# qcraftai/pillarnext

Measured on AMD Instinct MI355X. Metric: frames/s PillarNeXt-B nuScenes 300k-pt cloud (inference, end-to-end), higher is better.
Workload: dtype bf16

## Files before the change

include/pnx.h:

```cpp
#ifndef PNX_H
#define PNX_H

#include <stddef.h>
#include <stdint.h>

#ifdef __cplusplus
extern "C" {
#endif

typedef void* pnx_stream_t;

typedef enum pnx_status {
  PNX_OK = 0,
  PNX_ERR_INVALID = -1,
  PNX_ERR_UNSUPPORTED = -2,
  PNX_ERR_WORKSPACE = -3,
  PNX_ERR_HIP = -4
} pnx_status;

typedef enum pnx_dtype { PNX_F32 = 0, PNX_BF16 = 1, PNX_F16 = 2 } pnx_dtype;
typedef enum pnx_layout {
  PNX_NHWC = 0,
  PNX_NCHW = 1
} pnx_layout;
// ... 83 lines not shown

int pnx_bias_act_mask(const void* x, const void* residual, const float* bias, const uint8_t* mask, void* out, int64_t sites,
                      int32_t channels, int32_t dtype, int32_t relu, pnx_stream_t stream);
int pnx_sum_bias_act(const void* const* srcs, int32_t n_src, const float* bias, void* out, int64_t sites, int32_t channels, int32_t dtype,
                     int32_t relu, pnx_stream_t stream);
int pnx_deconv2x2_bf16(const void* x, const void* wfrag, const float* bias, void* y, int32_t batch, int32_t h, int32_t w, int32_t cin, int32_t cout,
                       int32_t relu, pnx_stream_t stream);
int pnx_deconv2x2_f16(const void* x, const void* wfrag, const float* bias, void* y, int32_t batch, int32_t h, int32_t w, int32_t cin, int32_t cout,
                       int32_t relu, pnx_stream_t stream);
int pnx_conv3x3_bf16(const void* x, const void* wfrag, const float* bias, const void* residual, const uint8_t* mask, void* y, int32_t batch,
                     int32_t h, int32_t w, int32_t cin, int32_t cout, int32_t stride, int32_t relu, uint8_t* row_dirty, const int32_t* tile_list,
                     const int32_t* tile_count, pnx_stream_t stream);
int pnx_conv3x3_f16(const void* x, const void* wfrag, const float* bias, const void* residual, const uint8_t* mask, void* y, int32_t batch,
                    int32_t h, int32_t w, int32_t cin, int32_t cout, int32_t stride, int32_t relu, uint8_t* row_dirty, const int32_t* tile_list,
                    const int32_t* tile_count, pnx_stream_t stream);
size_t pnx_conv3x3_wgrad_workspace_bytes(int32_t cin, int32_t cout);
int pnx_conv3x3_wgrad_bf16(const void* x, const void* dy, const uint8_t* mask, float* dw, int32_t batch, int32_t h, int32_t w, int32_t cin, int32_t cout,
                           int32_t stride, void* workspace, size_t workspace_bytes, pnx_stream_t stream);
int pnx_conv3x3_wgrad_x3(const void* x_hi, const void* x_lo, const void* dy_hi, const void* dy_lo, const uint8_t* mask, float* dw, int32_t batch, int32_t h,
                         int32_t w, int32_t cin, int32_t cout, int32_t stride, void* workspace, size_t workspace_bytes, pnx_stream_t stream);
int pnx_conv3x3_wgrad_x6(const void* x_hi, const void* x_mid, const void* x_lo, const void* dy_hi, const void* dy_mid, const void* dy_lo, const uint8_t* mask,
                         float* dw, int32_t batch, int32_t h, int32_t w, int32_t cin, int32_t cout, int32_t stride, void* workspace, size_t workspace_bytes,
                         pnx_stream_t stream);
int pnx_conv3x3_pack_weights(const void* w, int32_t dtype, int32_t cout, int32_t cin, int32_t transposed, void* wfrag, pnx_stream_t stream);
int pnx_conv3x3_tile_rows(int32_t cin, int32_t cout, int32_t stride);
int pnx_conv_tile_list(const uint8_t* mask, const uint8_t* const* row_dirty, int32_t n_dirty, int32_t batch, int32_t h, int32_t w, int32_t tile_rows,
                       int32_t* tile_list, int32_t* tile_count, pnx_stream_t stream);
int pnx_sephead_out_bf16(const void* x, const void* wfrag, const float* bias, void* y, int32_t batch, int32_t h, int32_t w, int32_t n_branch,
                         pnx_stream_t stream);
int pnx_sephead_out_f16(const void* x, const void* wfrag, const float* bias, void* y, int32_t batch, int32_t h, int32_t w, int32_t n_branch,
// ... 204 lines not shown
```

pillarnext_amd/_lib.py:

```python
import ctypes
import os

_HERE = os.path.dirname(os.path.abspath(__file__))
LIB_PATH = os.environ.get("PNX_LIB") or os.path.join(_HERE, "libpnx_hip.so")

PNX_F32, PNX_BF16, PNX_F16 = 0, 1, 2
PNX_NHWC, PNX_NCHW = 0, 1


class PnxError(RuntimeError):
    pass


class PnxGeom(ctypes.Structure):
    _fields_ = [("pc_min", ctypes.c_float * 3), ("voxel", ctypes.c_float * 3), ("gx", ctypes.c_int32), ("gy", ctypes.c_int32)]


PNX_GROUP_VOXEL, PNX_GROUP_PILLAR_CLAMP, PNX_GROUP_CYLINDER_CLAMP = 0, 1, 2


class PnxGroupGeom(ctypes.Structure):
    _fields_ = [("min", ctypes.c_float * 3), ("voxel", ctypes.c_float * 3), ("grid", ctypes.c_int32 * 3), ("mode", ctypes.c_int32),
                ("prefilter", ctypes.c_int32), ("keep_min", ctypes.c_float * 3), ("keep_max", ctypes.c_float * 3)]

# ... 56 lines not shown
    "pnx_deconv2x2_f16": (ctypes.c_int, [_vp, _vp, _vp, _vp, _i32, _i32, _i32, _i32, _i32, _i32, _vp]),
    "pnx_sephead_out_bf16": (ctypes.c_int, [_vp, _vp, _vp, _vp, _i32, _i32, _i32, _i32, _vp]),
    "pnx_sephead_out_f16": (ctypes.c_int, [_vp, _vp, _vp, _vp, _i32, _i32, _i32, _i32, _vp]),
    "pnx_masked_bn_blocks": (_i32, []),
    "pnx_masked_bn_reduce": (ctypes.c_int, [_vp, _i32, _i32, _vp, _vp]),
    "pnx_masked_bn_finalize": (ctypes.c_int, [_vp, _i32, _vp, _vp, _vp, ctypes.c_double, ctypes.c_double, _vp, _vp, _vp, _vp, _vp, _vp, _vp, _vp, _vp]),
    "pnx_masked_bn_bwd_finalize": (ctypes.c_int, [_vp, _vp, _i32, _vp, _vp, _vp, _vp, _vp, _vp]),
    "pnx_masked_bn_stats": (ctypes.c_int, [_vp, _i32, _vp, _i64, _i32, _vp, _vp, _vp]),
    "pnx_masked_bn_apply": (ctypes.c_int, [_vp, _vp, _i32, _vp, _i64, _i32, _vp, _vp, _i32, _vp, _vp]),
    "pnx_masked_bn_bwd_stats": (ctypes.c_int, [_vp, _vp, _vp, _i32, _vp, _i64, _i32, _vp, _vp, _vp, _vp, _i32, _vp, _vp]),
    "pnx_masked_bn_bwd_apply": (ctypes.c_int, [_vp, _vp, _vp, _i32, _vp, _i64, _i32, _vp, _vp, _vp, _vp, _i32, _vp, _vp, _vp, _vp, _vp]),
    "pnx_sephead_lazy_bf16": (ctypes.c_int, [_vp, _i32, _vp, _i32, _i32, _vp, _vp, _i32, _vp, _vp]),
    "pnx_sephead_lazy_f16": (ctypes.c_int, [_vp, _i32, _vp, _i32, _i32, _vp, _vp, _i32, _vp, _vp]),
    "pnx_conv3x3_bf16": (ctypes.c_int, [_vp, _vp, _vp, _vp, _vp, _vp, _i32, _i32, _i32, _i32, _i32, _i32, _i32, _vp, _vp, _vp, _vp]),
    "pnx_conv3x3_f16": (ctypes.c_int, [_vp, _vp, _vp, _vp, _vp, _vp, _i32, _i32, _i32, _i32, _i32, _i32, _i32, _vp, _vp, _vp, _vp]),
    "pnx_conv3x3_tile_rows": (ctypes.c_int, [_i32, _i32, _i32]),
    "pnx_conv3x3_pack_weights": (ctypes.c_int, [_vp, _i32, _i32, _i32, _i32, _vp, _vp]),
    "pnx_conv3x3_wgrad_workspace_bytes": (_sz, [_i32, _i32]),
    "pnx_conv3x3_wgrad_bf16": (ctypes.c_int, [_vp, _vp, _vp, _vp, _i32, _i32, _i32, _i32, _i32, _i32, _vp, _sz, _vp]),
    "pnx_conv3x3_wgrad_x3": (ctypes.c_int, [_vp, _vp, _vp, _vp, _vp, _vp, _i32, _i32, _i32, _i32, _i32, _i32, _vp, _sz, _vp]),
    "pnx_conv3x3_wgrad_x6": (ctypes.c_int, [_vp, _vp, _vp, _vp, _vp, _vp, _vp, _vp, _i32, _i32, _i32, _i32, _i32, _i32, _vp, _sz, _vp]),
    "pnx_conv3x3_dgrad_s2_bf16": (ctypes.c_int, [_vp, _vp, _vp, _vp, _i32, _i32, _i32, _i32, _i32, _vp]),
    "pnx_conv3x3_dgrad_s2_x3": (ctypes.c_int, [_vp, _vp, _vp, _vp, _vp, _vp, _i32, _i32, _i32, _i32, _i32, _vp]),
    "pnx_conv3x3_dgrad_s2_x6": (ctypes.c_int, [_vp, _vp, _vp, _vp, _vp, _vp, _vp, _vp, _i32, _i32, _i32, _i32, _i32, _vp]),
    "pnx_conv3x3_smallk": (ctypes.c_int, [_vp, _vp, _vp, _vp, _i32, _i32, _i32, _i32, _i32, _i32, _vp]),
    "pnx_conv3x3_smallk_wgrad_workspace_bytes": (_sz, [_i32]),
    "pnx_conv3x3_smallk_wgrad": (ctypes.c_int, [_vp, _vp, _vp, _vp, _i32, _i32, _i32, _i32, _i32, _i32, _vp, _sz, _vp]),
    "pnx_conv_tile_list": (ctypes.c_int, [_vp, _vp, _i32, _i32, _i32, _i32, _i32, _vp, _vp, _vp]),
    "pnx_mask_pool3": (ctypes.c_int, [_vp, _i32, _i32, _i32, _i32, _vp, _vp]),
    "pnx_split_f32": (ctypes.c_int, [_vp, _vp, _vp, _i64, _vp, _i32, _vp]),
    "pnx_conv3x3_x3": (ctypes.c_int, [_vp, _vp, _vp, _vp, _vp, _vp, _vp, _i32, _i32, _i32, _i32, _i32, _i32, _vp]),
# ... 96 lines not shown
```

pillarnext_amd/csrc/conv3x3.hip:

```cpp
#include "pnx_common.h"

namespace {

#include "conv_tile.h"

template <int CIN, int COUT, int STRIDE, bool W_LDS>
__global__ __launch_bounds__(256, 2) void k_conv3x3(const uint16_t* __restrict__ x, const uint4* __restrict__ wfrag,
                                                 const float* __restrict__ bias, const uint16_t* __restrict__ res,
                                                 const uint8_t* __restrict__ mask, uint16_t* __restrict__ y, int B, int H, int W, int Ho,
                                                 int Wo, int relu, uint8_t* __restrict__ row_dirty) {
  constexpr int CB = CIN / 16, MT = COUT / 32, KSTEPS = 9 * CB;
  constexpr int NT = (MT <= 2) ? 4 : 2;
  extern __shared__ uint4 s_w[];
  const int lane = threadIdx.x & 63, wv = threadIdx.x >> 6;
  const int px = lane & 31, kb = lane >> 5;
  if (W_LDS) {
    for (int i = threadIdx.x; i < KSTEPS * MT * 64; i += 256) s_w[i] = wfrag[i];
    __syncthreads();
  }
  const int tiles_x = (Wo + 31) >> 5, tiles_y = (Ho + NT - 1) / NT;
  const int64_t n_tiles = (int64_t)B * tiles_y * tiles_x;
  for (int64_t tile = (int64_t)blockIdx.x * 4 + wv; tile < n_tiles; tile += (int64_t)gridDim.x * 4) {
    const int tx = (int)(tile % tiles_x);
    const int ty = (int)((tile / tiles_x) % tiles_y);
// ... 267 lines not shown
  k_tile_list<<<(unsigned)((n_tiles + 15) / 16), 256, 0, st>>>(mask, ds, batch, h, w, tile_rows, tile_list, tile_count);
  PNX_LAUNCH_CHECK();
  return PNX_OK;
}
int pnx_conv_tile_list(const uint8_t* mask, const uint8_t* const* row_dirty, int32_t n_dirty, int32_t batch, int32_t h, int32_t w, int32_t tile_rows,
                       int32_t* tile_list, int32_t* tile_count, pnx_stream_t stream) {
  return conv_tile_list_impl(mask, row_dirty, n_dirty, batch, h, w, tile_rows, tile_list, tile_count, stream, true);
}
int pnx_conv_tile_list_prezeroed(const uint8_t* mask, const uint8_t* const* row_dirty, int32_t n_dirty, int32_t batch, int32_t h, int32_t w, int32_t tile_rows,
                                 int32_t* tile_list, int32_t* tile_count, pnx_stream_t stream) {
  return conv_tile_list_impl(mask, row_dirty, n_dirty, batch, h, w, tile_rows, tile_list, tile_count, stream, false);
}

#endif

int PNX_CONV_FN(pnx_conv3x3)(const void* x, const void* wfrag, const float* bias, const void* residual, const uint8_t* mask, void* y, int32_t batch,
                     int32_t h, int32_t w, int32_t cin, int32_t cout, int32_t stride, int32_t relu, uint8_t* row_dirty, const int32_t* tile_list,
                     const int32_t* tile_count, pnx_stream_t stream) {
  PNX_REQUIRE((tile_list == nullptr) == (tile_count == nullptr), PNX_ERR_INVALID, "tile_list and tile_count come together");
  PNX_REQUIRE(tile_list == nullptr || (mask != nullptr && pnx_conv3x3_tile_rows(cin, cout, stride) > 0), PNX_ERR_INVALID,
              "a tile list needs a mask and a kernel that takes one (pnx_conv3x3_tile_rows)");
  PNX_REQUIRE(x && wfrag && bias && y && batch > 0 && h > 0 && w > 0, PNX_ERR_INVALID, "bad arguments");
  PNX_REQUIRE(stride == 1 || stride == 2, PNX_ERR_UNSUPPORTED, "stride %d", stride);
  PNX_REQUIRE(row_dirty == nullptr || mask != nullptr, PNX_ERR_INVALID, "row_dirty needs an active-site mask");
  PNX_REQUIRE((((uintptr_t)x | (uintptr_t)y | (uintptr_t)wfrag | (uintptr_t)bias | (uintptr_t)residual) & 15) == 0, PNX_ERR_INVALID,
              "16-byte alignment required");
  const int ho = (h + 2 - 3) / stride + 1, wo = (w + 2 - 3) / stride + 1;
  hipStream_t st = (hipStream_t)stream;
  const ConvArgs a = {(const uint16_t*)x, (const uint4*)wfrag, bias, (const uint16_t*)residual, mask, (uint16_t*)y, batch, h, w, relu, row_dirty, tile_list,
                      tile_count, st};
  if (stride == 1 && getenv("PNX_CONV_DIRECT") == nullptr) {
    static const int pc_mode = getenv("PNX_CONV_PC") != nullptr ? atoi(getenv("PNX_CONV_PC")) : 1;
    static const int pack_mode = getenv("PNX_CONV_PACK") != nullptr ? atoi(getenv("PNX_CONV_PACK")) : 3;
    if (pc_mode != 0) {
      if (cin == 64 && cout == 64) return launch_pc<64, 64>(a, (pack_mode & 2) != 0);
      if (residual == nullptr && (pc_mode & 4)) {
        if (cin == 64 && cout == 320) return launch_pc<64, 320>(a);
        if (cin == 64 && cout == 384) return launch_pc<64, 384>(a);
        if (cin == 64 && cout == 448) return launch_pc<64, 448>(a);
      }
      if (pc_mode & 2) {
        if (cin == 128 && cout == 128) return launch_pc<128, 128>(a);
        if (cin == 256 && cout == 256) return launch_pc<256, 256>(a);
      }
    }
    if (cin == 64 && cout == 64) return launch_lds<64>(a);
    const bool pack = (pack_mode & 1) != 0;
    if (cin == 128 && cout == 128) return launch_ldsx<128, 128>(a, pack);
    if (cin == 256 && cout == 64) return launch_ldsx<256, 64>(a);
    if (cin == 256 && cout == 256) return launch_ldsx<256, 256>(a, pack);
// ... 5 lines not shown
    if (cin == 64 && cout == 128) return launch_s2<64, 128, 1>(x, wfrag, bias, mask, y, batch, h, w, ho, wo, relu, row_dirty, st);
    if (cin == 128 && cout == 256) return launch_s2<128, 256, 1>(x, wfrag, bias, mask, y, batch, h, w, ho, wo, relu, row_dirty, st);
    if (cin == 256 && cout == 256) return launch_s2<256, 256, 1>(x, wfrag, bias, mask, y, batch, h, w, ho, wo, relu, row_dirty, st);
  }
#define PNX_CONV_CASE(CI, CO)                             \
  if (cin == CI && cout == CO) {                          \
    if (stride == 1) return launch<CI, CO, 1>(a, ho, wo); \
    return launch<CI, CO, 2>(a, ho, wo);                  \
  }
  PNX_CONV_CASE(64, 64)
  PNX_CONV_CASE(64, 128)
  PNX_CONV_CASE(128, 128)
#undef PNX_CONV_CASE
  pnx_set_error("pnx_conv3x3: no kernel for %d -> %d channels", cin, cout);
  return PNX_ERR_UNSUPPORTED;
}

#ifndef PNX_CONV_F16
}
namespace {
#include "conv_dgrad_s2.h"

template <int NP>
int dgrad_s2_impl(const char* name, PnxPieces<NP> g, PnxPieces<NP> wfrag_t, const uint8_t* mask_in, void* dx, int32_t batch, int32_t h, int32_t w, int32_t cin,
                  int32_t cout, pnx_stream_t stream) {
  PNX_REQUIRE(g.complete() && wfrag_t.complete() && mask_in && dx && batch > 0 && h > 0 && w > 0, PNX_ERR_INVALID, "%s: bad arguments", name);
  PNX_REQUIRE(((g.bits() | wfrag_t.bits() | (uintptr_t)dx) & 15) == 0, PNX_ERR_INVALID, "16-byte alignment required");
  hipStream_t st = (hipStream_t)stream;
  if (cin == 64 && cout == 128) return launch_dgrad_s2<128, 64, NP>(g, wfrag_t, mask_in, dx, batch, h, w, st);
  if (cin == 128 && cout == 256) return launch_dgrad_s2<256, 128, NP>(g, wfrag_t, mask_in, dx, batch, h, w, st);
// ... 94 lines not shown
```

pillarnext_amd/csrc/conv_pc.h:

```cpp
#pragma once

__device__ __forceinline__ void pc_barrier_lds() { asm volatile("s_waitcnt lgkmcnt(0)\n\ts_barrier" ::: "memory"); }
__device__ __forceinline__ void pc_barrier_all() { asm volatile("s_waitcnt vmcnt(0) lgkmcnt(0)\n\ts_barrier" ::: "memory"); }

#ifdef PNX_CONV_TIMERS
#define PC_T_DECL unsigned long long pc_T[8] = {0, 0, 0, 0, 0, 0, 0, 0}; unsigned long long pc_tk = __builtin_amdgcn_s_memtime();
#define PC_TOCK(k)                                               \
  {                                                              \
    const unsigned long long _n = __builtin_amdgcn_s_memtime();  \
    pc_T[k] += _n - pc_tk;                                       \
    pc_tk = _n;                                                  \
  }
#define PC_T_FLUSH                                                   \
  if ((threadIdx.x & 63) == 0) {                                     \
    for (int k = 0; k < 8; k++) atomicAdd(&g_conv_T[k], pc_T[k]);    \
  }
#else
#define PC_T_DECL
#define PC_TOCK(k)
#define PC_T_FLUSH
#endif

template <int NR, int CIN, int COUT, bool HAS_RES, int NRG, int NSLOT, int SLOT_N, int NP = 1>
__device__ __forceinline__ void pc_rows(const uint4* __restrict__ s_ring, int& g, const uint4* __restrict__ wfrag, const uint4* __restrict__ wfrag2,
// ... 148 lines not shown
      transpose_row32(pk, lane);
      int l = lane;
      asm volatile("" : "+v"(l));
      const int cj = code(j);
#pragma unroll
      for (int d = 0; d < 2; d++) {
        const int P = 16 * d + (l >> 2);
        const int pc = __builtin_amdgcn_ds_bpermute(P << 2, cj);
        if (P < n_g[j]) *reinterpret_cast<uint4*>(yp + pc_pix_off64(pc, W) + (uint32_t)((l & 3) * 16)) = pk[d];
      }
    }
  }
  PC_TOCK(3)
}

template <int CIN, int COUT, bool HAS_RES, int NP = 1, bool PACK = false>
__global__ __launch_bounds__(768, 3) void k_conv3x3_pc(const uint16_t* __restrict__ x, const uint16_t* __restrict__ x2, const uint4* __restrict__ wfrag,
                                                       const uint4* __restrict__ wfrag2, const float* __restrict__ bias,
                                                       const uint16_t* __restrict__ res, const uint8_t* __restrict__ mask, uint16_t* __restrict__ y,
                                                       int B, int H, int W, int relu, uint8_t* __restrict__ row_dirty, int slot,
                                                       const int32_t* __restrict__ tlist, const int32_t* __restrict__ tcount,
                                                       const uint16_t* __restrict__ x3 = nullptr, const uint4* __restrict__ wfrag3 = nullptr) {
  constexpr bool X3 = NP == 2, F32 = NP > 1;
  constexpr int TH = CIN == 64 ? 16 : 8;
  constexpr int NRG = TH / 4, NCG = 8 / NRG, PASS_C = NCG * 32, NPASS = COUT / PASS_C, NSLAB = CIN / 64;
  constexpr int NSLOT = CIN == 64 ? 2 : 3, DEPTH = NSLOT - 1;
  constexpr int NFILL = F32 ? NPASS * NSLAB * NP : CIN == 64 ? 1 : NPASS * NSLAB;
  constexpr int YS = F32 ? 2 : 1;
  static_assert(!F32 || (!HAS_RES && (CIN > 64 || NPASS == 1)), "fp32 product: no residual; one pass when the tile is filled once per source");
  constexpr int SLOT_N = (TH + 2) * LDS_HW * 8;
  static_assert(COUT % PASS_C == 0 && CIN % 64 == 0, "passes of NCG x 32 output channels over 64-channel input slabs");
  static_assert(!PACK || (CIN == 64 && COUT == 64 && NP == 1), "the packed-pixel form serves the bf16 / f16 64 -> 64 layers");
  __shared__ uint4 s_ring[NSLOT * SLOT_N];
  __shared__ uint16_t s_list[PACK ? 4 * TH * 32 : 1];
  __shared__ int4 s_tile[4];
  __shared__ uint32_t s_rowmask[4][TH];
  __shared__ int4 s_drow[4][NRG];
  __shared__ uint4 s_dmask[4][NRG];
// ... 10 lines not shown
#pragma unroll
    for (int i = 0; i < 5; i++) {
      const int col = 8 * i + (lane >> 3), k = lane & 7;
      colv[i] = col;
      voff[i] = (uint32_t)(col * CIN + ((k ^ lds_swz(col)) * 8)) * 2u;
    }
    typedef __attribute__((address_space(1))) const void* gptr_t;
    typedef __attribute__((address_space(3))) void* lptr_t;

    auto tile_index = [&](int n) -> int64_t {
      const int64_t idx = (n < 3 || slot < 0) ? (int64_t)blockIdx.x + (int64_t)n * gridDim.x : (int64_t)s_tick[n & 3] + 3 * (int64_t)gridDim.x;
      return tile_at(tlist, idx, n_tiles);
    };
    uint32_t mb[TH / 2];
    uint32_t dirty = 0;
    auto load_meta = [&](int64_t t) {
#pragma unroll
      for (int k = 0; k < TH / 2; k++) mb[k] = 0;
      dirty = 0;
      if (t < 0) return;
      const int tx = (int)(t % tiles_x), ty = (int)((t / tiles_x) % tiles_y), b = (int)(t / ((int64_t)tiles_x * tiles_y));
      const int ox = tx * 32 + (lane & 31);
#pragma unroll
      for (int k = 0; k < TH / 2; k++) {
        const int oy = ty * TH + 2 * k + (lane >> 5);
        if (ox < W && oy < H) mb[k] = mask != nullptr ? (uint32_t)mask[((int64_t)b * H + oy) * W + ox] : 1u;
      }
      const int oy2 = ty * TH + lane;
      if (lane < TH && oy2 < H) dirty = row_dirty != nullptr ? (uint32_t)row_dirty[((int64_t)b * H + oy2) * tiles_x + tx] : 1u;
    };

    int n = 0, f = 0, nf = 0, g = 0;
    int64_t t_next = tile_index(0);
    load_meta(t_next);
    int cb = 0, cy0 = 0, cx0 = 0;
    uint32_t am = 0;

    auto advance = [&]() -> bool {
      const int64_t t = t_next;
      if (t < 0) {
        if (pw == 0 && lane == 0) s_tile[n & 3] = make_int4(-1, 0, 0, 0);
        return false;
      }
      const int tx = (int)(t % tiles_x), ty = (int)((t / tiles_x) % tiles_y);
// ... 4 lines not shown
      int n_px = 0;
#pragma unroll
      for (int k = 0; k < TH / 2; k++) {
        const unsigned long long bal = __ballot(mb[k] != 0);
        const uint32_t lo = (uint32_t)bal, hi = (uint32_t)(bal >> 32);
        if constexpr (PACK) {
          if (pw == 0 && mb[k] != 0)
            s_list[(n & 3) * (TH * 32) + n_px + __popcll(bal & ((1ull << lane) - 1ull))] = (uint16_t)(((2 * k + (lane >> 5)) << 5) | (lane & 31));
          n_px += __popcll(bal);
        }
        if (lane == 2 * k) my_rm = lo;
        if (lane == 2 * k + 1) my_rm = hi;
        am |= (lo != 0 ? 1u : 0u) << (2 * k) | (hi != 0 ? 1u : 0u) << (2 * k + 1);
      }
      const uint32_t was = (uint32_t)__ballot(dirty != 0) & ((1u << TH) - 1u);
      if (pw == 0) {
        if (lane < TH) s_rowmask[n & 3][lane] = my_rm;
        if (lane == 0) s_tile[n & 3] = make_int4(cb, cy0, cx0, (int)(am | (uint32_t)n_px << 16));
        if (lane < NRG * 4) {
          uint32_t rest = am;
          for (int k = 0; k < lane && rest; k++) rest &= rest - 1;
          const int row = rest != 0 ? __builtin_ctz(rest) : -1;
          const uint32_t m = row >= 0 ? s_rowmask[n & 3][row] : 0u;
          reinterpret_cast<int*>(&s_drow[n & 3][lane % NRG])[lane / NRG] = row;
          reinterpret_cast<uint32_t*>(&s_dmask[n & 3][lane % NRG])[lane / NRG] = m;
        }
      }
      if (slot >= 0 && pw == 0 && lane == 0) s_tick[(n + 3) & 3] = atomicAdd(&g_tile_ctr[slot][0], 1u);
      t_next = tile_index(n + 1);
      load_meta(t_next);
// ... 28 lines not shown
      n++;
      return true;
    };

    auto next_fill = [&]() -> bool {
      if (f == nf && !advance()) return false;
      if (am != 0) {
        const int sl = f % NSLAB;
        uint4* dstslot = s_ring + (g % NSLOT) * SLOT_N;
        const uint16_t* xs = X3 && (f / NSLAB) % 2 == 1 ? x2 : x;
        if constexpr (NP == 3) {
          const int q = (f / NSLAB) % 3;
          xs = q == 0 ? x3 : q == 1 ? x2 : x;
        }
        const uint16_t* xt = xs + (((int64_t)cb * H + (cy0 - 1)) * W + (cx0 - 1)) * CIN + 64 * sl;
        bool col_ok[5];
#pragma unroll
        for (int i = 0; i < 5; i++) col_ok[i] = (unsigned)(cx0 - 1 + colv[i]) < (unsigned)W && (i < 4 || lane < 16);
#pragma unroll 1
        for (int r = pw; r < TH + 2; r += 4) {
          const int iy = cy0 - 1 + r;
          const bool row_ok = iy >= 0 && iy < H;
          const char* rowp = reinterpret_cast<const char*>(xt + (int64_t)r * W * CIN);
#pragma unroll
          for (int i = 0; i < 5; i++) {
            if (row_ok && col_ok[i]) {
              __builtin_amdgcn_global_load_lds((gptr_t)(rowp + voff[i]), (lptr_t)(dstslot + r * LDS_HW * 8 + 64 * i), 16, 0, 0);
            } else if (i < 4 || lane < 16) {
              dstslot[r * LDS_HW * 8 + 64 * i + lane] = make_uint4(0, 0, 0, 0);
            }
          }
        }
      }
      f++;
      g++;
// ... 95 lines not shown
      default: PC_ROWS(4); break;
    }
#undef PC_ROWS
  }
  if (threadIdx.x == 0) sched_done(slot);
  PC_T_FLUSH
}

template <int CIN, int COUT>
int launch_pc(const ConvArgs& a, bool pack = false) {
  constexpr int TH = CIN == 64 ? 16 : 8;
  int64_t nb = (int64_t)a.B * ((a.H + TH - 1) / TH) * ((a.W + 31) / 32);
  if (nb > 256) nb = 256;
  const int slot = a.mask != nullptr ? next_sched_slot() : -1;
  if constexpr (CIN == 64 && COUT == 64) {
    if (pack && a.mask != nullptr) {
      if (a.res != nullptr)
        k_conv3x3_pc<64, 64, true, 1, true><<<(unsigned)nb, 768, 0, a.st>>>(a.x, nullptr, a.wfrag, nullptr, a.bias, a.res, a.mask, a.y, a.B, a.H, a.W, a.relu,
                                                                          a.row_dirty, slot, a.tlist, a.tcount);
      else
        k_conv3x3_pc<64, 64, false, 1, true><<<(unsigned)nb, 768, 0, a.st>>>(a.x, nullptr, a.wfrag, nullptr, a.bias, nullptr, a.mask, a.y, a.B, a.H, a.W, a.relu,
                                                                           a.row_dirty, slot, a.tlist, a.tcount);
      PNX_LAUNCH_CHECK();
      return PNX_OK;
    }
  }
  if (a.res != nullptr)
    k_conv3x3_pc<CIN, COUT, true><<<(unsigned)nb, 768, 0, a.st>>>(a.x, nullptr, a.wfrag, nullptr, a.bias, a.res, a.mask, a.y, a.B, a.H, a.W, a.relu, a.row_dirty,
                                                                slot, a.tlist, a.tcount);
  else
// ... 19 lines not shown
```

pillarnext_amd/csrc/conv_tile.h:

```cpp
#pragma once

typedef float v16f __attribute__((ext_vector_type(16)));
typedef float f32x2 __attribute__((ext_vector_type(2)));

#ifdef PNX_CONV_F16
typedef _Float16 el8 __attribute__((ext_vector_type(8)));
typedef _Float16 el2 __attribute__((ext_vector_type(2)));
#define PNX_MFMA32(a, b, c) __builtin_amdgcn_mfma_f32_32x32x16_f16(a, b, c, 0, 0, 0)
#define PNX_MFMA16(a, b, c) __builtin_amdgcn_mfma_f32_16x16x32_f16(a, b, c, 0, 0, 0)
#define PNX_CONV_FN(name) name##_f16
__device__ __forceinline__ uint32_t el_lo_bits(uint32_t w) { return __float_as_uint((float)__builtin_bit_cast(el2, w)[0]); }
__device__ __forceinline__ uint32_t el_hi_bits(uint32_t w) { return __float_as_uint((float)__builtin_bit_cast(el2, w)[1]); }
#else
typedef __bf16 el8 __attribute__((ext_vector_type(8)));
typedef __bf16 el2 __attribute__((ext_vector_type(2)));
#define PNX_MFMA32(a, b, c) __builtin_amdgcn_mfma_f32_32x32x16_bf16(a, b, c, 0, 0, 0)
#define PNX_MFMA16(a, b, c) __builtin_amdgcn_mfma_f32_16x16x32_bf16(a, b, c, 0, 0, 0)
#define PNX_CONV_FN(name) name##_bf16
__device__ __forceinline__ uint32_t el_lo_bits(uint32_t w) { return w << 16; }
__device__ __forceinline__ uint32_t el_hi_bits(uint32_t w) { return w & 0xffff0000u; }
#endif
__device__ __forceinline__ uint32_t pack_el(float lo, float hi) {
  const f32x2 v = {lo, hi};
  return __builtin_bit_cast(uint32_t, __builtin_convertvector(v, el2));
// ... 147 lines not shown
      }
    }
}

struct ConvArgs {
  const uint16_t* x;
  const uint4* wfrag;
  const float* bias;
  const uint16_t* res;
  const uint8_t* mask;
  uint16_t* y;
  int B, H, W, relu;
  uint8_t* row_dirty;
  const int32_t *tlist, *tcount;
  hipStream_t st;
};
```

pillarnext_amd/csrc/enqueue.hip:

```cpp
#include "pnx_common.h"

extern "C" int pnx_conv_tile_list_prezeroed(const uint8_t* mask, const uint8_t* const* row_dirty, int32_t n_dirty, int32_t batch, int32_t h, int32_t w,
                                            int32_t tile_rows, int32_t* tile_list, int32_t* tile_count, pnx_stream_t stream);

namespace {

__global__ __launch_bounds__(256) void k_lazy_cells(const int64_t* __restrict__ order, const int32_t* __restrict__ seg_len, const int64_t* __restrict__ list_key_off,
                                                    int32_t pre_max, int64_t n, int64_t* __restrict__ local) {
  const int64_t i = (int64_t)blockIdx.x * blockDim.x + threadIdx.x;
  if (i >= n) return;
  const int64_t s = i / pre_max;
  const int32_t j = (int32_t)(i - s * pre_max);
  local[i] = j < seg_len[s] ? order[i] - list_key_off[s] : 0;
}

struct ZeroRanges {
  uint32_t* p[8];
  int64_t end[8];
  int n;
};
__global__ __launch_bounds__(256) void k_zero_ranges(ZeroRanges z) {
  const int64_t total = z.end[z.n - 1];
  for (int64_t i = (int64_t)blockIdx.x * 256 + threadIdx.x; i < total; i += (int64_t)gridDim.x * 256) {
    int r = 0;
// ... 14 lines not shown
  z.p[z.n] = (uint32_t*)p;
  z.end[z.n] = (z.n ? z.end[z.n - 1] : 0) + words;
  z.n++;
}

int run_op(const pnx_op& o, hipStream_t st) {
  const int32_t* i = o.i;
  const void* const* p = o.p;
  switch (o.kind) {
    case PNX_OP_MASK_POOL3:
      return pnx_mask_pool3((const uint8_t*)p[0], i[0], i[1], i[2], i[3], (uint8_t*)p[1], st);
    case PNX_OP_TILE_LIST:
      PNX_REQUIRE(i[0] >= 0 && i[0] <= 8, PNX_ERR_INVALID, "tile list over %d row_dirty arrays (at most 8)", i[0]);
      return pnx_conv_tile_list_prezeroed((const uint8_t*)p[0], (const uint8_t* const*)&p[3], i[0], i[1], i[2], i[3], i[4], (int32_t*)p[1], (int32_t*)p[2], st);
    case PNX_OP_CONV3X3:
      return (i[7] == PNX_F16 ? pnx_conv3x3_f16 : pnx_conv3x3_bf16)(p[0], p[1], (const float*)p[2], p[3], (const uint8_t*)p[4], (void*)p[5], i[0], i[1], i[2],
                                                                    i[3], i[4], i[5], i[6], (uint8_t*)p[6], (const int32_t*)p[7], (const int32_t*)p[8], st);
    case PNX_OP_DECONV2X2:
      return (i[6] == PNX_F16 ? pnx_deconv2x2_f16 : pnx_deconv2x2_bf16)(p[0], p[1], (const float*)p[2], (void*)p[3], i[0], i[1], i[2], i[3], i[4], i[5], st);
    case PNX_OP_SEPHEAD_OUT:
      return (i[4] == PNX_F16 ? pnx_sephead_out_f16 : pnx_sephead_out_bf16)(p[0], p[1], (const float*)p[2], (void*)p[3], i[0], i[1], i[2], i[3], st);
    default:
      pnx_set_error("unknown op kind %d", o.kind);
      return PNX_ERR_INVALID;
  }
}

}

extern "C" int pnx_enqueue(const pnx_op* ops, int32_t n_ops, pnx_stream_t stream) {
  PNX_REQUIRE(ops != nullptr && n_ops >= 0, PNX_ERR_INVALID, "pnx_enqueue: bad arguments");
  hipStream_t st = (hipStream_t)stream;
// ... 81 lines not shown
```

pillarnext_amd/models.py:

```python
import copy
import inspect
import os
import weakref

import numpy as np

import torch
import torch.nn.functional as F
from torch import nn

from . import ops
from .plan import Dyn, LaunchPlan


def _spconv_weight_to_conv2d(w, conv):
    want = tuple(conv.weight.shape)
    co, ci, kh, kw = want
    layout = getattr(conv, "assume_layout", None)
    if layout == "dense":
        if tuple(w.shape) != want:
            raise RuntimeError(f"dense-layout checkpoint holds {tuple(w.shape)} for Conv2d {want}")
        return w
    if layout == "spconv":
        if tuple(w.shape) != (co, kh, kw, ci):
# ... 951 lines not shown
            y = F.conv2d(x, self.weight, None, self.stride, self.padding, self.dilation)
        if not y.is_contiguous(memory_format=torch.channels_last):
            y = y.contiguous(memory_format=torch.channels_last)
        if post_residual is not None:
            return ops.bias_act_mask_(y, self.bias, mask, post_residual, 2 if self.relu else 0)
        return ops.bias_act_mask_(y, self.bias, mask, residual, self.relu)


class _HipConv3x3(nn.Module):

    def __init__(self, weight, bias, stride=1, dtype=torch.bfloat16):
        super().__init__()
        self.cout, self.cin, self.stride = weight.shape[0], weight.shape[1], int(stride)
        self.register_buffer("wfrag", ops.conv3x3_pack_weights(weight, dtype=dtype))
        self.register_buffer("bias", bias.float().contiguous())
    def forward(self, x, mask=None, residual=None, out=None, tiles=None, plan=None):
        call = ops.conv3x3_masked if plan is None else plan.conv3x3
        return call(x, self.wfrag, self.bias, self.cout, self.stride, mask, residual, True, out=out, tiles=tiles if self.stride == 1 else None)


class _HipDeconv2x2(nn.Module):

    def __init__(self, weight, bias, relu=True, dtype=torch.bfloat16):
        super().__init__()
        self.cout, self.relu = weight.shape[1], relu
        self.register_buffer("wfrag", ops.deconv2x2_pack_weights(weight, dtype=dtype))
        self.register_buffer("bias", bias.float().contiguous())

    def forward(self, x, mask=None, residual=None, out=None, plan=None):
        if plan is None:
            return ops.deconv2x2(x, self.wfrag, self.bias, self.cout, self.relu)
        return plan.deconv2x2(x, self.wfrag, self.bias, self.cout, out, self.relu)

# ... 68 lines not shown
        return getattr(self.pend, name)


class FusedPillarNeXt(nn.Module):

    def __init__(self, det, dtype=torch.bfloat16, hip_conv=None):
        super().__init__()
        import os

        if hip_conv is None:
            hip_conv = os.environ.get("PNX_HIP_CONV", "1") != "0"
        self._ws = {}
        self.use_plan = os.environ.get("PNX_PLAN", "1") != "0"
        self.sparse_ws = os.environ.get("PNX_SPARSE_WS", "1") != "0"
        self.tile_lists = os.environ.get("PNX_TILE_LISTS", "1") != "0"
        self.decode_on_side_stream = os.environ.get("PNX_DECODE_STREAM", "1") != "0"
        self.reader = det.reader
        self.post_processing = det.post_processing
        self.head_ref = det.head
        self.dtype = dtype
        self._decoder = None
        bb = det.backbone
        self.stages = nn.ModuleList()
        self.stage_meta = []
        for blk in bb.blocks:
            mods = nn.ModuleList()
            first = blk[0]
            w, b = _fold_bn(first.conv.weight, first.norm)
            mods.append(_backbone_conv(w, b, first.stride, first.kernel_size // 2, dtype, hip_conv))
            for rb in list(blk)[1:]:
# ... 143 lines not shown
            if lazy:
                packed_out.append(LazyTask(t, up))
            elif packed_out is not None:
                packed_out.append(t)
            else:
                d, o = {}, 0
                for nme, k in zip(names, outs_n):
                    d[nme] = t[:, o:o + k]
                    o += k
                preds.append(d)
        mark("head")
        return preds

    def _backbone(self, x, mask, plan=None, mark=lambda name: None, taps=None):
        for si, (mods, (stride, subm)) in enumerate(zip(self.stages, self.stage_meta)):
            if not subm:
                mask = ops.mask_pool3(mask, stride) if plan is None else plan.mask_pool3(mask, ops.mask_pool3_out(mask, stride), stride)
            ws, k = self._stage_workspace(si, mods, mask), 0
            tiles = self._stage_tiles(si, mods, mask, ws, plan)

            def run(m, inp, res=None):
                nonlocal k
                if ws is None or not isinstance(m, _HipConv3x3):
                    assert plan is None
                    return m(inp, mask, residual=res)
                k += 1
                return m(inp, mask, residual=res, out=ws[(k - 1) % 3], tiles=tiles, plan=plan)

            x = run(mods[0], x)
            for j in range(1, len(mods), 2):
                y = run(mods[j], x)
                x = run(mods[j + 1], y, x)
            mark(f"backbone.stage{si}")
            if taps is not None:
                taps[f"stage{si}"] = x
        return x, mask

    def _head(self, x, lazy, plan=None):
        c1s, c2s = (self.lazy_conv1, self.lazy_conv2) if lazy else (self.task_conv1, self.task_conv2)

        def run(m, inp, out):
            return m(inp) if plan is None else m(inp, out=out, plan=plan)

        o_sh, outs = None, [(None, None, None)] * len(c1s)
        if plan is not None:
            def new(c, s):
                return torch.empty((x.shape[0], c, s * x.shape[2], s * x.shape[3]), dtype=self.dtype, device=x.device, memory_format=torch.channels_last)
# ... 173 lines not shown
```

pillarnext_amd/ops.py:

```python
import ctypes

import torch

from . import _lib
from ._lib import PNX_BF16, PNX_F16, PNX_F32, PNX_NCHW, PNX_NHWC, PnxError, check, lib, ptr, stream_ptr

_DT = {torch.float32: PNX_F32, torch.bfloat16: PNX_BF16, torch.float16: PNX_F16}


def _need_cuda(t, name):
    if not t.is_cuda:
        raise PnxError(f"{name} must be a CUDA (ROCm) tensor; the PillarNeXt hot path has no CPU implementation")
    if not t.is_contiguous():
        raise PnxError(f"{name} must be contiguous")


class Workspace:

    def __init__(self):
        self.buf = None

    def get(self, nbytes, device):
        if self.buf is None or self.buf.numel() < nbytes or self.buf.device != device:
            self.buf = torch.empty(int(nbytes * 1.25) + 256, dtype=torch.uint8, device=device)
# ... 614 lines not shown

def _conv3x3_dims(x, wfrag, cout, stride, mask, residual, out, cuda=False):
    xs = _half_nhwc(x, "conv3x3", cuda=cuda)
    if wfrag.dtype != xs.dtype or (residual is not None and _like(residual).dtype != xs.dtype):
        raise PnxError("conv3x3: weights / residual of another dtype than the input")
    B, ci, H, W = xs.shape
    Ho, Wo = _out_hw(H, W, stride)
    if out is not None:
        y, dirty = out
        if (tuple(_half_nhwc(y, "conv3x3 output", xs.dtype).shape) != (B, cout, Ho, Wo)
                or (dirty is not None and (mask is None or tuple(dirty.shape) != (B, Ho, (Wo + 31) // 32)))):
            raise PnxError("conv3x3: output / workspace of the wrong shape (a workspace needs a mask)")
    return B, H, W, ci, _DT[xs.dtype], Ho, Wo


def conv3x3_masked(x, wfrag, bias, cout, stride=1, mask=None, residual=None, relu=True, out=None, tiles=None):
    B, H, W, ci, _, Ho, Wo = _conv3x3_dims(x, wfrag, cout, stride, mask, residual, out, cuda=True)
    y, dirty = out if out is not None else (torch.empty((B, cout, Ho, Wo), dtype=x.dtype, device=x.device, memory_format=torch.channels_last), None)
    tl, tc = tiles if tiles is not None else (None, None)
    check(_conv_fn("conv3x3", x.dtype)(ptr(x), ptr(wfrag), ptr(bias), ptr(residual), ptr(mask), ptr(y), B, H, W, ci, cout, stride, 1 if relu else 0,
                                       ptr(dirty), ptr(tl), ptr(tc), stream_ptr()), "pnx_conv3x3")
    return y


def _i3(v):
    return (ctypes.c_int32 * 3)(*[int(a) for a in v])


class Sp3Index:

    def __init__(self, batch, grid, device):
        self.batch, self.grid = int(batch), tuple(int(g) for g in grid)
        self.nbytes = lib().pnx_sp3_index_bytes(self.batch, _i3(self.grid))
        if self.nbytes == 0:
            raise PnxError(f"sparse3d: bad grid {self.batch} x {self.grid}")
        self.buf = torch.empty((self.nbytes,), dtype=torch.uint8, device=device)
# ... 354 lines not shown
```

pillarnext_amd/plan.py:

```python
import ctypes

from . import ops
from ._lib import PnxError, check, lib, stream_ptr

OP_MASK_POOL3, OP_TILE_LIST, OP_CONV3X3, OP_DECONV2X2, OP_SEPHEAD_OUT = 1, 2, 3, 4, 5


class PnxOp(ctypes.Structure):
    _fields_ = [("kind", ctypes.c_int32), ("i", ctypes.c_int32 * 9), ("p", ctypes.c_void_p * 11)]


assert ctypes.sizeof(PnxOp) == 128, "pnx_op layout drifted (include/pnx.h)"


class Dyn:

    def __init__(self, name, like):
        self.name, self.like = name, like


class LaunchPlan:
    def __init__(self):
        self._ops, self._keep, self._dyn, self._arr = [], [], {}, None

# ... 16 lines not shown
                op.p[k] = a.data_ptr()
                self._keep.append(a)
        self._ops.append(op)

    def mask_pool3(self, mask_in, mask_out, stride):
        self._add(OP_MASK_POOL3, [*ops._like(mask_in).shape, stride], [mask_in, ops.mask_pool3_out(mask_in, stride, mask_out)])
        return mask_out

    def tile_list(self, mask, dirties, tile_rows, out):
        if len(dirties) > 8:
            raise PnxError("tile_list: an entry has room for 8 row_dirty arrays")
        tl, tc = ops.conv_tile_buffers(mask, tile_rows, out)
        self._add(OP_TILE_LIST, [len(dirties), *ops._like(mask).shape, tile_rows], [mask, tl, tc] + list(dirties))
        return out

    def conv3x3(self, x, wfrag, bias, cout, stride=1, mask=None, residual=None, relu=True, out=None, tiles=None):
        B, H, W, ci, dt, _, _ = ops._conv3x3_dims(x, wfrag, cout, stride, mask, residual, out)
        tl, tc = tiles if tiles is not None else (None, None)
        self._add(OP_CONV3X3, [B, H, W, ci, cout, stride, 1 if relu else 0, dt], [x, wfrag, bias, residual, mask, *out, tl, tc])
        return out[0]

    def deconv2x2(self, x, wfrag, bias, cout, y, relu=True):
        B, H, W, ci, dt = ops._conv_dims("deconv2x2", x, wfrag, y, cout, 2)
        self._add(OP_DECONV2X2, [B, H, W, ci, cout, 1 if relu else 0, dt], [x, wfrag, bias, y])
        return y

    def sephead_out(self, x, wfrag, bias, y):
        B, H, W, ci, dt = ops._conv_dims("sephead_out", x, wfrag, y, 16, 1)
        self._add(OP_SEPHEAD_OUT, [B, H, W, ci // 64, dt], [x, wfrag, bias, y])
        return y

    def freeze(self):
        self._arr = (PnxOp * max(len(self._ops), 1))(*self._ops)
        self._bound = {}
# ... 23 lines not shown
```

Measured before the change: 758.8.

## Skip gathering inactive input pixels in stage-0 64->64 sparse conv via input mask

Adds an input active-site mask path to the 64->64 pillar conv kernel. Halo pixels whose input is inactive are zero-filled in LDS instead of loaded from global memory, and whole input rows that no active output row needs are skipped. This is meant to cut redundant global-to-LDS traffic for sparse stage-0 feature maps, at the cost of an extra mask read and ballots per tile. The row-skip part also applies to the existing non-input-mask path, but the input-mask path is wired only for stage 0 and is disabled by default through PNX_STAGE0_IN_MASK=0.

Result: no change. 761.6 (median of 6 runs) (+0.4%).

```diff
diff --git a/include/pnx.h b/include/pnx.h
--- a/include/pnx.h
+++ b/include/pnx.h
@@ -121,6 +121,12 @@
 int pnx_conv3x3_f16(const void* x, const void* wfrag, const float* bias, const void* residual, const uint8_t* mask, void* y, int32_t batch,
                     int32_t h, int32_t w, int32_t cin, int32_t cout, int32_t stride, int32_t relu, uint8_t* row_dirty, const int32_t* tile_list,
                     const int32_t* tile_count, pnx_stream_t stream);
+int pnx_conv3x3_in_bf16(const void* x, const void* wfrag, const float* bias, const void* residual, const uint8_t* mask, const uint8_t* in_mask, void* y,
+                        int32_t batch, int32_t h, int32_t w, int32_t cin, int32_t cout, int32_t stride, int32_t relu, uint8_t* row_dirty,
+                        const int32_t* tile_list, const int32_t* tile_count, pnx_stream_t stream);
+int pnx_conv3x3_in_f16(const void* x, const void* wfrag, const float* bias, const void* residual, const uint8_t* mask, const uint8_t* in_mask, void* y,
+                       int32_t batch, int32_t h, int32_t w, int32_t cin, int32_t cout, int32_t stride, int32_t relu, uint8_t* row_dirty,
+                       const int32_t* tile_list, const int32_t* tile_count, pnx_stream_t stream);
 size_t pnx_conv3x3_wgrad_workspace_bytes(int32_t cin, int32_t cout);
 int pnx_conv3x3_wgrad_bf16(const void* x, const void* dy, const uint8_t* mask, float* dw, int32_t batch, int32_t h, int32_t w, int32_t cin, int32_t cout,
                            int32_t stride, void* workspace, size_t workspace_bytes, pnx_stream_t stream);
diff --git a/pillarnext_amd/_lib.py b/pillarnext_amd/_lib.py
--- a/pillarnext_amd/_lib.py
+++ b/pillarnext_amd/_lib.py
@@ -94,7 +94,9 @@
     "pnx_sephead_lazy_f16": (ctypes.c_int, [_vp, _i32, _vp, _i32, _i32, _vp, _vp, _i32, _vp, _vp]),
     "pnx_conv3x3_bf16": (ctypes.c_int, [_vp, _vp, _vp, _vp, _vp, _vp, _i32, _i32, _i32, _i32, _i32, _i32, _i32, _vp, _vp, _vp, _vp]),
     "pnx_conv3x3_f16": (ctypes.c_int, [_vp, _vp, _vp, _vp, _vp, _vp, _i32, _i32, _i32, _i32, _i32, _i32, _i32, _vp, _vp, _vp, _vp]),
-    "pnx_conv3x3_tile_rows": (ctypes.c_int, [_i32, _i32, _i32]),
+    "pnx_conv3x3_in_bf16": (ctypes.c_int, [_vp, _vp, _vp, _vp, _vp, _vp, _vp, _i32, _i32, _i32, _i32, _i32, _i32, _i32, _vp, _vp, _vp, _vp]),
+    "pnx_conv3x3_in_f16": (ctypes.c_int, [_vp, _vp, _vp, _vp, _vp, _vp, _vp, _i32, _i32, _i32, _i32, _i32, _i32, _i32, _vp, _vp, _vp, _vp]),
+    "pnx_conv3x3_tile_rows":(ctypes.c_int, [_i32, _i32, _i32]),
     "pnx_conv3x3_pack_weights": (ctypes.c_int, [_vp, _i32, _i32, _i32, _i32, _vp, _vp]),
     "pnx_conv3x3_wgrad_workspace_bytes": (_sz, [_i32, _i32]),
     "pnx_conv3x3_wgrad_bf16": (ctypes.c_int, [_vp, _vp, _vp, _vp, _i32, _i32, _i32, _i32, _i32, _i32, _vp, _sz, _vp]),
diff --git a/pillarnext_amd/csrc/conv3x3.hip b/pillarnext_amd/csrc/conv3x3.hip
--- a/pillarnext_amd/csrc/conv3x3.hip
+++ b/pillarnext_amd/csrc/conv3x3.hip
@@ -305,10 +305,11 @@
 
 #endif
 
-int PNX_CONV_FN(pnx_conv3x3)(const void* x, const void* wfrag, const float* bias, const void* residual, const uint8_t* mask, void* y, int32_t batch,
-                     int32_t h, int32_t w, int32_t cin, int32_t cout, int32_t stride, int32_t relu, uint8_t* row_dirty, const int32_t* tile_list,
-                     const int32_t* tile_count, pnx_stream_t stream) {
+int PNX_CONV_FN(pnx_conv3x3_in)(const void* x, const void* wfrag, const float* bias, const void* residual, const uint8_t* mask, const uint8_t* in_mask,
+                        void* y, int32_t batch, int32_t h, int32_t w, int32_t cin, int32_t cout, int32_t stride, int32_t relu, uint8_t* row_dirty,
+                        const int32_t* tile_list, const int32_t* tile_count, pnx_stream_t stream) {
   PNX_REQUIRE((tile_list == nullptr) == (tile_count == nullptr), PNX_ERR_INVALID, "tile_list and tile_count come together");
+  PNX_REQUIRE(in_mask == nullptr || mask != nullptr, PNX_ERR_INVALID, "in_mask needs an active-site mask");
   PNX_REQUIRE(tile_list == nullptr || (mask != nullptr && pnx_conv3x3_tile_rows(cin, cout, stride) > 0), PNX_ERR_INVALID,
               "a tile list needs a mask and a kernel that takes one (pnx_conv3x3_tile_rows)");
   PNX_REQUIRE(x && wfrag && bias && y && batch > 0 && h > 0 && w > 0, PNX_ERR_INVALID, "bad arguments");
@@ -319,12 +320,17 @@
   const int ho = (h + 2 - 3) / stride + 1, wo = (w + 2 - 3) / stride + 1;
   hipStream_t st = (hipStream_t)stream;
   const ConvArgs a = {(const uint16_t*)x, (const uint4*)wfrag, bias, (const uint16_t*)residual, mask, (uint16_t*)y, batch, h, w, relu, row_dirty, tile_list,
-                      tile_count, st};
+                      tile_count, st, nullptr};
   if (stride == 1 && getenv("PNX_CONV_DIRECT") == nullptr) {
     static const int pc_mode = getenv("PNX_CONV_PC") != nullptr ? atoi(getenv("PNX_CONV_PC")) : 1;
     static const int pack_mode = getenv("PNX_CONV_PACK") != nullptr ? atoi(getenv("PNX_CONV_PACK")) : 3;
     if (pc_mode != 0) {
-      if (cin == 64 && cout == 64) return launch_pc<64, 64>(a, (pack_mode & 2) != 0);
+      if (cin == 64 && cout == 64) {
+        static const bool use_in_mask = getenv("PNX_CONV_IN_MASK") == nullptr || atoi(getenv("PNX_CONV_IN_MASK")) != 0;
+        ConvArgs ai = a;
+        ai.in_mask = use_in_mask ? in_mask : nullptr;
+        return launch_pc<64, 64>(ai, (pack_mode & 2) != 0);
+      }
       if (residual == nullptr && (pc_mode & 4)) {
         if (cin == 64 && cout == 320) return launch_pc<64, 320>(a);
         if (cin == 64 && cout == 384) return launch_pc<64, 384>(a);
@@ -360,6 +366,12 @@
 #undef PNX_CONV_CASE
   pnx_set_error("pnx_conv3x3: no kernel for %d -> %d channels", cin, cout);
   return PNX_ERR_UNSUPPORTED;
+}
+
+int PNX_CONV_FN(pnx_conv3x3)(const void* x, const void* wfrag, const float* bias, const void* residual, const uint8_t* mask, void* y, int32_t batch,
+                     int32_t h, int32_t w, int32_t cin, int32_t cout, int32_t stride, int32_t relu, uint8_t* row_dirty, const int32_t* tile_list,
+                     const int32_t* tile_count, pnx_stream_t stream) {
+  return PNX_CONV_FN(pnx_conv3x3_in)(x, wfrag, bias, residual, mask, nullptr, y, batch, h, w, cin, cout, stride, relu, row_dirty, tile_list, tile_count, stream);
 }
 
 #ifndef PNX_CONV_F16
diff --git a/pillarnext_amd/csrc/conv_pc.h b/pillarnext_amd/csrc/conv_pc.h
--- a/pillarnext_amd/csrc/conv_pc.h
+++ b/pillarnext_amd/csrc/conv_pc.h
@@ -186,14 +186,16 @@
   PC_TOCK(3)
 }
 
-template <int CIN, int COUT, bool HAS_RES, int NP = 1, bool PACK = false>
+template <int CIN, int COUT, bool HAS_RES, int NP = 1, bool PACK = false, bool INM = false>
 __global__ __launch_bounds__(768, 3) void k_conv3x3_pc(const uint16_t* __restrict__ x, const uint16_t* __restrict__ x2, const uint4* __restrict__ wfrag,
                                                        const uint4* __restrict__ wfrag2, const float* __restrict__ bias,
                                                        const uint16_t* __restrict__ res, const uint8_t* __restrict__ mask, uint16_t* __restrict__ y,
                                                        int B, int H, int W, int relu, uint8_t* __restrict__ row_dirty, int slot,
                                                        const int32_t* __restrict__ tlist, const int32_t* __restrict__ tcount,
-                                                       const uint16_t* __restrict__ x3 = nullptr, const uint4* __restrict__ wfrag3 = nullptr) {
+                                                       const uint16_t* __restrict__ x3 = nullptr, const uint4* __restrict__ wfrag3 = nullptr,
+                                                       const uint8_t* __restrict__ in_mask = nullptr) {
   constexpr bool X3 = NP == 2, F32 = NP > 1;
+  static_assert(!INM || (CIN == 64 && COUT == 64 && NP == 1), "the input's active set is used by the bf16 / f16 64 -> 64 layers");
   constexpr int TH = CIN == 64 ? 16 : 8;
   constexpr int NRG = TH / 4, NCG = 8 / NRG, PASS_C = NCG * 32, NPASS = COUT / PASS_C, NSLAB = CIN / 64;
   constexpr int NSLOT = CIN == 64 ? 2 : 3, DEPTH = NSLOT - 1;
@@ -234,10 +236,17 @@
     };
     uint32_t mb[TH / 2];
     uint32_t dirty = 0;
+    constexpr int NIR = INM ? (TH + 2 + 3) / 4 : 1;
+    [[maybe_unused]] uint32_t ib[NIR];
+    [[maybe_unused]] unsigned long long iw[NIR];
     auto load_meta = [&](int64_t t) {
 #pragma unroll
       for (int k = 0; k < TH / 2; k++) mb[k] = 0;
       dirty = 0;
+      if constexpr (INM) {
+#pragma unroll
+        for (int j = 0; j < NIR; j++) ib[j] = 0;
+      }
       if (t < 0) return;
       const int tx = (int)(t % tiles_x), ty = (int)((t / tiles_x) % tiles_y), b = (int)(t / ((int64_t)tiles_x * tiles_y));
       const int ox = tx * 32 + (lane & 31);
@@ -248,6 +257,14 @@
       }
       const int oy2 = ty * TH + lane;
       if (lane < TH && oy2 < H) dirty = row_dirty != nullptr ? (uint32_t)row_dirty[((int64_t)b * H + oy2) * tiles_x + tx] : 1u;
+      if constexpr (INM) {
+        const int ix = tx * 32 - 1 + lane;
+#pragma unroll
+        for (int j = 0; j < NIR; j++) {
+          const int r = pw + 4 * j, iy = ty * TH - 1 + r;
+          if (r < TH + 2 && lane < 34 && (unsigned)ix < (unsigned)W && (unsigned)iy < (unsigned)H) ib[j] = (uint32_t)in_mask[((int64_t)b * H + iy) * W + ix];
+        }
+      }
     };
 
     int n = 0, f = 0, nf = 0, g = 0;
@@ -282,6 +299,20 @@
         am |= (lo != 0 ? 1u : 0u) << (2 * k) | (hi != 0 ? 1u : 0u) << (2 * k + 1);
       }
       const uint32_t was = (uint32_t)__ballot(dirty != 0) & ((1u << TH) - 1u);
+      if constexpr (INM) {
+#pragma unroll
+        for (int j = 0; j < NIR; j++) iw[j] = __ballot(ib[j] != 0);
+        const uint32_t need = am | am << 1 | am << 2;
+        uint4* dstslot = s_ring + (g % NSLOT) * SLOT_N;
+#pragma unroll
+        for (int j = 0; j < NIR; j++) {
+          const int r = pw + 4 * j;
+          if (r >= TH + 2 || ((need >> r) & 1u) == 0) continue;
+#pragma unroll
+          for (int i = 0; i < 5; i++)
+            if (((iw[j] >> colv[i]) & 1ull) == 0 && (i < 4 || lane < 16)) dstslot[r * LDS_HW * 8 + 64 * i + lane] = make_uint4(0, 0, 0, 0);
+        }
+      }
       if (pw == 0) {
         if (lane < TH) s_rowmask[n & 3][lane] = my_rm;
         if (lane == 0) s_tile[n & 3] = make_int4(cb, cy0, cx0, (int)(am | (uint32_t)n_px << 16));
@@ -340,11 +371,28 @@
           xs = q == 0 ? x3 : q == 1 ? x2 : x;
         }
         const uint16_t* xt = xs + (((int64_t)cb * H + (cy0 - 1)) * W + (cx0 - 1)) * CIN + 64 * sl;
+        const uint32_t need = CIN == 64 && NP == 1 ? am | am << 1 | am << 2 : 0xffffffffu;
+        if constexpr (INM) {
+#pragma unroll
+          for (int j = 0; j < NIR; j++) {
+            const int r = pw + 4 * j;
+            if (r >= TH + 2 || ((need >> r) & 1u) == 0 || iw[j] == 0) continue;
+            const char* rowp = reinterpret_cast<const char*>(xt + (int64_t)r * W * CIN);
+#pragma unroll
+            for (int i = 0; i < 5; i++)
+              if ((iw[j] >> colv[i]) & 1ull)
+                __builtin_amdgcn_global_load_lds((gptr_t)(rowp + voff[i]), (lptr_t)(dstslot + r * LDS_HW * 8 + 64 * i), 16, 0, 0);
+          }
+          f++;
+          g++;
+          return true;
+        }
         bool col_ok[5];
 #pragma unroll
         for (int i = 0; i < 5; i++) col_ok[i] = (unsigned)(cx0 - 1 + colv[i]) < (unsigned)W && (i < 4 || lane < 16);
 #pragma unroll 1
         for (int r = pw; r < TH + 2; r += 4) {
+          if (((need >> r) & 1u) == 0) continue;
           const int iy = cy0 - 1 + r;
           const bool row_ok = iy >= 0 && iy < H;
           const char* rowp = reinterpret_cast<const char*>(xt + (int64_t)r * W * CIN);
@@ -470,6 +518,19 @@
   if (nb > 256) nb = 256;
   const int slot = a.mask != nullptr ? next_sched_slot() : -1;
   if constexpr (CIN == 64 && COUT == 64) {
+    if (a.in_mask != nullptr && a.mask != nullptr) {
+#define PC_INM(RES_, PACK_)                                                                                                                                  \
+  k_conv3x3_pc<64, 64, RES_, 1, PACK_, true><<<(unsigned)nb, 768, 0, a.st>>>(a.x, nullptr, a.wfrag, nullptr, a.bias, RES_ ? a.res : nullptr, a.mask, a.y, a.B, a.H, \
+                                                                             a.W, a.relu, a.row_dirty, slot, a.tlist, a.tcount, nullptr, nullptr, a.in_mask)
+      if (a.res != nullptr) {
+        if (pack) PC_INM(true, true); else PC_INM(true, false);
+      } else {
+        if (pack) PC_INM(false, true); else PC_INM(false, false);
+      }
+#undef PC_INM
+      PNX_LAUNCH_CHECK();
+      return PNX_OK;
+    }
     if (pack && a.mask != nullptr) {
       if (a.res != nullptr)
         k_conv3x3_pc<64, 64, true, 1, true><<<(unsigned)nb, 768, 0, a.st>>>(a.x, nullptr, a.wfrag, nullptr, a.bias, a.res, a.mask, a.y, a.B, a.H, a.W, a.relu,
diff --git a/pillarnext_amd/csrc/conv_tile.h b/pillarnext_amd/csrc/conv_tile.h
--- a/pillarnext_amd/csrc/conv_tile.h
+++ b/pillarnext_amd/csrc/conv_tile.h
@@ -185,4 +185,5 @@
   uint8_t* row_dirty;
   const int32_t *tlist, *tcount;
   hipStream_t st;
+  const uint8_t* in_mask;
 };
diff --git a/pillarnext_amd/csrc/enqueue.hip b/pillarnext_amd/csrc/enqueue.hip
--- a/pillarnext_amd/csrc/enqueue.hip
+++ b/pillarnext_amd/csrc/enqueue.hip
@@ -52,8 +52,9 @@
       PNX_REQUIRE(i[0] >= 0 && i[0] <= 8, PNX_ERR_INVALID, "tile list over %d row_dirty arrays (at most 8)", i[0]);
       return pnx_conv_tile_list_prezeroed((const uint8_t*)p[0], (const uint8_t* const*)&p[3], i[0], i[1], i[2], i[3], i[4], (int32_t*)p[1], (int32_t*)p[2], st);
     case PNX_OP_CONV3X3:
-      return (i[7] == PNX_F16 ? pnx_conv3x3_f16 : pnx_conv3x3_bf16)(p[0], p[1], (const float*)p[2], p[3], (const uint8_t*)p[4], (void*)p[5], i[0], i[1], i[2],
-                                                                    i[3], i[4], i[5], i[6], (uint8_t*)p[6], (const int32_t*)p[7], (const int32_t*)p[8], st);
+      return (i[7] == PNX_F16 ? pnx_conv3x3_in_f16 : pnx_conv3x3_in_bf16)(p[0], p[1], (const float*)p[2], p[3], (const uint8_t*)p[4], (const uint8_t*)p[9],
+                                                                          (void*)p[5], i[0], i[1], i[2], i[3], i[4], i[5], i[6], (uint8_t*)p[6],
+                                                                          (const int32_t*)p[7], (const int32_t*)p[8], st);
     case PNX_OP_DECONV2X2:
       return (i[6] == PNX_F16 ? pnx_deconv2x2_f16 : pnx_deconv2x2_bf16)(p[0], p[1], (const float*)p[2], (void*)p[3], i[0], i[1], i[2], i[3], i[4], i[5], st);
     case PNX_OP_SEPHEAD_OUT:
diff --git a/pillarnext_amd/models.py b/pillarnext_amd/models.py
--- a/pillarnext_amd/models.py
+++ b/pillarnext_amd/models.py
@@ -989,9 +989,10 @@
         self.cout, self.cin, self.stride = weight.shape[0], weight.shape[1], int(stride)
         self.register_buffer("wfrag", ops.conv3x3_pack_weights(weight, dtype=dtype))
         self.register_buffer("bias", bias.float().contiguous())
-    def forward(self, x, mask=None, residual=None, out=None, tiles=None, plan=None):
+    def forward(self, x, mask=None, residual=None, out=None, tiles=None, plan=None, in_mask=None):
         call = ops.conv3x3_masked if plan is None else plan.conv3x3
-        return call(x, self.wfrag, self.bias, self.cout, self.stride, mask, residual, True, out=out, tiles=tiles if self.stride == 1 else None)
+        extra = {"in_mask": in_mask} if in_mask is not None and self.stride == 1 else {}
+        return call(x, self.wfrag, self.bias, self.cout, self.stride, mask, residual, True, out=out, tiles=tiles if self.stride == 1 else None, **extra)
 
 
 class _HipDeconv2x2(nn.Module):
@@ -1090,6 +1091,7 @@
         self.use_plan = os.environ.get("PNX_PLAN", "1") != "0"
         self.sparse_ws = os.environ.get("PNX_SPARSE_WS", "1") != "0"
         self.tile_lists = os.environ.get("PNX_TILE_LISTS", "1") != "0"
+        self.stage0_in_mask = os.environ.get("PNX_STAGE0_IN_MASK", "0") != "0"
         self.decode_on_side_stream = os.environ.get("PNX_DECODE_STREAM", "1") != "0"
         self.reader = det.reader
         self.post_processing = det.post_processing
@@ -1263,23 +1265,25 @@
 
     def _backbone(self, x, mask, plan=None, mark=lambda name: None, taps=None):
         for si, (mods, (stride, subm)) in enumerate(zip(self.stages, self.stage_meta)):
+            mask_in = mask
             if not subm:
                 mask = ops.mask_pool3(mask, stride) if plan is None else plan.mask_pool3(mask, ops.mask_pool3_out(mask, stride), stride)
             ws, k = self._stage_workspace(si, mods, mask), 0
             tiles = self._stage_tiles(si, mods, mask, ws, plan)
 
-            def run(m, inp, res=None):
+            def run(m, inp, res=None, active=None):
                 nonlocal k
                 if ws is None or not isinstance(m, _HipConv3x3):
                     assert plan is None
                     return m(inp, mask, residual=res)
                 k += 1
-                return m(inp, mask, residual=res, out=ws[(k - 1) % 3], tiles=tiles, plan=plan)
-
-            x = run(mods[0], x)
+                return m(inp, mask, residual=res, out=ws[(k - 1) % 3], tiles=tiles, plan=plan, in_mask=active)
+
+            a_in, a_blk = (mask_in, mask) if self.stage0_in_mask and si == 0 and stride == 1 else (None, None)
+            x = run(mods[0], x, active=a_in)
             for j in range(1, len(mods), 2):
-                y = run(mods[j], x)
-                x = run(mods[j + 1], y, x)
+                y = run(mods[j], x, active=a_blk)
+                x = run(mods[j + 1], y, x, active=a_blk)
             mark(f"backbone.stage{si}")
             if taps is not None:
                 taps[f"stage{si}"] = x
diff --git a/pillarnext_amd/ops.py b/pillarnext_amd/ops.py
--- a/pillarnext_amd/ops.py
+++ b/pillarnext_amd/ops.py
@@ -652,12 +652,20 @@
     return B, H, W, ci, _DT[xs.dtype], Ho, Wo
 
 
-def conv3x3_masked(x, wfrag, bias, cout, stride=1, mask=None, residual=None, relu=True, out=None, tiles=None):
+def _conv3x3_in_mask(in_mask, mask, B, H, W):
+    if in_mask is not None:
+        m = _like(in_mask)
+        if mask is None or m.dtype != torch.uint8 or tuple(m.shape) != (B, H, W) or not m.is_contiguous():
+            raise PnxError("conv3x3: in_mask must be a contiguous uint8 (B,H,W) map and needs a mask")
+    return in_mask
+
+
+def conv3x3_masked(x, wfrag, bias, cout, stride=1, mask=None, residual=None, relu=True, out=None, tiles=None, in_mask=None):
     B, H, W, ci, _, Ho, Wo = _conv3x3_dims(x, wfrag, cout, stride, mask, residual, out, cuda=True)
     y, dirty = out if out is not None else (torch.empty((B, cout, Ho, Wo), dtype=x.dtype, device=x.device, memory_format=torch.channels_last), None)
     tl, tc = tiles if tiles is not None else (None, None)
-    check(_conv_fn("conv3x3", x.dtype)(ptr(x), ptr(wfrag), ptr(bias), ptr(residual), ptr(mask), ptr(y), B, H, W, ci, cout, stride, 1 if relu else 0,
-                                       ptr(dirty), ptr(tl), ptr(tc), stream_ptr()), "pnx_conv3x3")
+    check(_conv_fn("conv3x3_in", x.dtype)(ptr(x), ptr(wfrag), ptr(bias), ptr(residual), ptr(mask), ptr(_conv3x3_in_mask(in_mask, mask, B, H, W)), ptr(y), B, H, W,
+                                          ci, cout, stride, 1 if relu else 0, ptr(dirty), ptr(tl), ptr(tc), stream_ptr()), "pnx_conv3x3")
     return y
 
 
diff --git a/pillarnext_amd/plan.py b/pillarnext_amd/plan.py
--- a/pillarnext_amd/plan.py
+++ b/pillarnext_amd/plan.py
@@ -54,10 +54,11 @@
         self._add(OP_TILE_LIST, [len(dirties), *ops._like(mask).shape, tile_rows], [mask, tl, tc] + list(dirties))
         return out
 
-    def conv3x3(self, x, wfrag, bias, cout, stride=1, mask=None, residual=None, relu=True, out=None, tiles=None):
+    def conv3x3(self, x, wfrag, bias, cout, stride=1, mask=None, residual=None, relu=True, out=None, tiles=None, in_mask=None):
         B, H, W, ci, dt, _, _ = ops._conv3x3_dims(x, wfrag, cout, stride, mask, residual, out)
         tl, tc = tiles if tiles is not None else (None, None)
-        self._add(OP_CONV3X3, [B, H, W, ci, cout, stride, 1 if relu else 0, dt], [x, wfrag, bias, residual, mask, *out, tl, tc])
+        self._add(OP_CONV3X3, [B, H, W, ci, cout, stride, 1 if relu else 0, dt],
+                  [x, wfrag, bias, residual, mask, *out, tl, tc, ops._conv3x3_in_mask(in_mask, mask, B, H, W)])
         return out[0]
 
     def deconv2x2(self, x, wfrag, bias, cout, y, relu=True):
```
